# huziqi/NALO-SLAM

Hardware: AMD Instinct MI355X
Metric: keyframes/sec, KITTI-00 dense 8-KF photometric BA; pose RMSE vs ref (higher is better)
Workload: dtype f32; 1 GPU; kitti00_8kf; image=1224x368, levels=4, window_frames=8, active_points=2000, residuals=14000, tracked_frames_per_keyframe=3, multi_gpu=replicas (window too small to shard)

## Files before the change

### nalo-slam_amd/csrc/kernels_trk_lm.hip

```cpp
#include "nalo_internal.h"
#include <hip/hip_ext.h>
#include "reduce.h"
#include "trk_device.h"

namespace nalo {

constexpr int kLmThreads = 512;
constexpr int kLmStride = 56;

struct TrkLmParams {
    TrkLevel lv[NALO_MAX_LEVELS];
    double T0[12], aff0[2], ref_aff[2], minRes[5];
    float expRef, expNew;
    int coarsest, has_minres, stop_lvl, have_repeated_in;
    double* out;
    double seq;
    unsigned long long* partial;
    unsigned tag0;
};

struct LmState {
    double T[12], aff[2];
    double Tn[12], affn[2];
    double H[64], b[8], resOld[6], resNew[6];
    double lastRes[5], flow[3];
    float RKi[9], t[3], Ki[9], affa, affb, b0, cutoff, maxEnergy;
    float lambda, levelCutoffRepeat;
    int lvl, it, phase, haveRepeated, good, evals, done, break_pending, next_lvl;
    int evals_lvl[NALO_MAX_LEVELS];
};

__device__ __forceinline__ void lm_se3_exp(const double (&xi)[8], double (&T)[12]) {
    const double wx = xi[3], wy = xi[4], wz = xi[5];
    const double th2 = wx * wx + wy * wy + wz * wz;
    double qi, qr, a, bq;
    if (th2 < 0.25) {
        const double u = 0.25 * th2;
        double sc = -1.0 / 121645100408832000.0, cc = 1.0 / 6402373705728000.0;
        sc = sc * u + 1.0 / 355687428096000.0; cc = cc * u - 1.0 / 20922789888000.0;
        sc = sc * u - 1.0 / 1307674368000.0;   cc = cc * u + 1.0 / 87178291200.0;
        sc = sc * u + 1.0 / 6227020800.0;      cc = cc * u - 1.0 / 479001600.0;
        sc = sc * u - 1.0 / 39916800.0;        cc = cc * u + 1.0 / 3628800.0;
        sc = sc * u + 1.0 / 362880.0;          cc = cc * u - 1.0 / 40320.0;
        sc = sc * u - 1.0 / 5040.0;            cc = cc * u + 1.0 / 720.0;
        sc = sc * u + 1.0 / 120.0;             cc = cc * u - 1.0 / 24.0;
        sc = sc * u - 1.0 / 6.0;               cc = cc * u + 0.5;
        sc = sc * u + 1.0;                     cc = 1.0 - cc * u;
        qi = 0.5 * sc; qr = cc;
        const double v = th2;
        double pa = -1.0 / 51090942171709440000.0, pb = 1.0 / 1124000727777607680000.0;
        pa = pa * v + 1.0 / 121645100408832000.0; pb = pb * v - 1.0 / 2432902008176640000.0;
        pa = pa * v - 1.0 / 355687428096000.0;    pb = pb * v + 1.0 / 6402373705728000.0;
        pa = pa * v + 1.0 / 1307674368000.0;      pb = pb * v - 1.0 / 20922789888000.0;
        pa = pa * v - 1.0 / 6227020800.0;         pb = pb * v + 1.0 / 87178291200.0;
        pa = pa * v + 1.0 / 39916800.0;           pb = pb * v - 1.0 / 479001600.0;
        pa = pa * v - 1.0 / 362880.0;             pb = pb * v + 1.0 / 3628800.0;
        pa = pa * v + 1.0 / 5040.0;               pb = pb * v - 1.0 / 40320.0;
        pa = pa * v - 1.0 / 120.0;                pb = pb * v + 1.0 / 720.0;
        pa = pa * v + 1.0 / 6.0;                  pb = pb * v - 1.0 / 24.0;
        bq = pa; a = pb * v + 0.5;
    } else {
        const double th = sqrt(th2);
        double sh, ch;
        sincos(0.5 * th, &sh, &ch);
        qi = sh / th; qr = ch;
        a = (2.0 * sh * sh) / th2; bq = (th - 2.0 * sh * ch) / (th2 * th);
    }
    double q[4] = {qr, qi * wx, qi * wy, qi * wz};
    const double qn2 = q[0] * q[0] + q[1] * q[1] + q[2] * q[2] + q[3] * q[3];
    const double qs = 1.5 - 0.5 * qn2;
#pragma unroll
    for (int i = 0; i < 4; ++i) q[i] *= qs;
    const double w = q[0], x = q[1], y = q[2], z = q[3];
    const double R[9] = {1 - 2 * (y * y + z * z), 2 * (x * y - w * z), 2 * (x * z + w * y), 2 * (x * y + w * z), 1 - 2 * (x * x + z * z), 2 * (y * z - w * x),
                         2 * (x * z - w * y), 2 * (y * z + w * x), 1 - 2 * (x * x + y * y)};
    const double O[9] = {0, -wz, wy, wz, 0, -wx, -wy, wx, 0};
    double O2[9], V[9];
#pragma unroll
    for (int i = 0; i < 3; ++i)
#pragma unroll
        for (int j = 0; j < 3; ++j) O2[i * 3 + j] = O[i * 3] * O[j] + O[i * 3 + 1] * O[3 + j] + O[i * 3 + 2] * O[6 + j];
#pragma unroll
    for (int i = 0; i < 9; ++i) V[i] = ((i % 4 == 0) ? 1.0 : 0.0) + a * O[i] + bq * O2[i];
#pragma unroll
    for (int i = 0; i < 3; ++i) {
#pragma unroll
        for (int j = 0; j < 3; ++j) T[i * 4 + j] = R[i * 3 + j];
        T[i * 4 + 3] = V[i * 3] * xi[0] + V[i * 3 + 1] * xi[1] + V[i * 3 + 2] * xi[2];
    }
}
__device__ __forceinline__ void lm_se3_mul(const double (&A)[12], const double (&B)[12], double (&C)[12]) {
#pragma unroll
    for (int i = 0; i < 3; ++i) {
#pragma unroll
        for (int j = 0; j < 3; ++j) C[i * 4 + j] = A[i * 4] * B[j] + A[i * 4 + 1] * B[4 + j] + A[i * 4 + 2] * B[8 + j];
        C[i * 4 + 3] = A[i * 4] * B[3] + A[i * 4 + 1] * B[7] + A[i * 4 + 2] * B[11] + A[i * 4 + 3];
    }
}
__device__ __forceinline__ double lm_bcast(double v, int srclane) {
    const int lo = __builtin_amdgcn_readlane(__double2loint(v), srclane), hi = __builtin_amdgcn_readlane(__double2hiint(v), srclane);
    return __hiloint2double(hi, lo);
}
__device__ __forceinline__ void lm_wave_sync() {
    __builtin_amdgcn_fence(__ATOMIC_RELEASE, "wavefront");
    __builtin_amdgcn_wave_barrier();
    __builtin_amdgcn_fence(__ATOMIC_ACQUIRE, "wavefront");
}
__device__ __forceinline__ constexpr int lm_ut(int r, int c) { return r * 8 - r * (r - 1) / 2 + (c - r); }
__device__ __forceinline__ void lm_ldlt8_uniform(double (&U)[36], const double (&rhs)[8], double (&x)[8]) {
    double dinv[8];
#pragma unroll
    for (int k = 0; k < 8; ++k) {
        const double d = U[lm_ut(k, k)];
        const bool ok = d != 0.0 && isfinite(d);
        double rd = __builtin_amdgcn_rcp(d);
        rd = rd * (2.0 - d * rd); rd = rd * (2.0 - d * rd);
        dinv[k] = ok ? rd : 0.0;
#pragma unroll
        for (int i = k + 1; i < 8; ++i) {
            const double l = U[lm_ut(k, i)] * dinv[k];
#pragma unroll
            for (int j = i; j < 8; ++j) U[lm_ut(i, j)] -= l * U[lm_ut(k, j)];
            U[lm_ut(k, i)] = l;
        }
    }
    double y[8];
#pragma unroll
    for (int i = 0; i < 8; ++i) {
        double sacc = rhs[i];
#pragma unroll
        for (int j = 0; j < i; ++j) sacc -= U[lm_ut(j, i)] * y[j];
        y[i] = sacc;
    }
#pragma unroll
    for (int i = 7; i >= 0; --i) {
        double sacc = y[i] * dinv[i];
#pragma unroll
        for (int j = i + 1; j < 8; ++j) sacc -= U[lm_ut(i, j)] * x[j];
        x[i] = sacc;
    }
}

__device__ __forceinline__ void lm_prepare_eval(LmState& S, const TrkLmParams& P, int lvl, float levelCutoffRepeat, const double (&T)[12], double aff0, double aff1, bool write) {
    const TrkLevel& L = P.lv[lvl];
    float expF = P.expRef, expT = P.expNew;
    if (expF == 0 || expT == 0) expT = expF = 1;
    const double a = exp(aff0 - P.ref_aff[0]) * expT / expF, bq = aff1 - a * P.ref_aff[1];
    const float Ki[9] = {1.0f / L.fx, 0, -L.cx / L.fx, 0, 1.0f / L.fy, -L.cy / L.fy, 0, 0, 1};
    float Rf[9], RKi[9];
#pragma unroll
    for (int i = 0; i < 3; ++i)
#pragma unroll
        for (int j = 0; j < 3; ++j) Rf[i * 3 + j] = (float)T[i * 4 + j];
#pragma unroll
    for (int i = 0; i < 3; ++i)
#pragma unroll
        for (int j = 0; j < 3; ++j) RKi[i * 3 + j] = Rf[i * 3] * Ki[j] + Rf[i * 3 + 1] * Ki[3 + j] + Rf[i * 3 + 2] * Ki[6 + j];
    if (!write) return;
    S.affa = (float)a; S.affb = (float)bq; S.b0 = (float)P.ref_aff[1];
#pragma unroll
    for (int i = 0; i < 9; ++i) { S.RKi[i] = RKi[i]; S.Ki[i] = Ki[i]; }
#pragma unroll
    for (int i = 0; i < 3; ++i) S.t[i] = (float)T[i * 4 + 3];
    S.cutoff = kCoarseCutoffTH * levelCutoffRepeat;
    S.maxEnergy = 2 * kHuberTH * S.cutoff - kHuberTH * kHuberTH;
}
__device__ __forceinline__ double lm_scale(int r) { return r < 3 ? (double)kScaleXiRot : r < 6 ? (double)kScaleXiTrans : r == 6 ? (double)kScaleA : (double)kScaleB; }
__device__ __forceinline__ int lm_max_iterations(int lvl) { return lvl == 0 ? 10 : lvl == 1 ? 20 : 50; }
__device__ __forceinline__ unsigned long long lm_pack(float v, unsigned tag) { return ((unsigned long long)tag << 32) | (unsigned long long)__float_as_uint(v); }

__global__ __launch_bounds__(kLmThreads) void trk_lm_kernel(TrkLmParams P) {
    __shared__ float rows[(kLmThreads / 4) * kLmStride];
    __shared__ double sums[64];
    __shared__ double part[kLmThreads / 64][64];
    __shared__ LmState S;
    __shared__ int bar_ok;
    const int tid = threadIdx.x, blk = blockIdx.x, NB = gridDim.x;
    const float lambdaExtrapolationLimit = 0.001f;
    int timed_out = 0;
    if (tid == 0) bar_ok = 1;
    float c_id = 0.f, c_x = 0.f, c_y = 0.f, c_rc = 0.f;
    int cached_lvl = -1;

    if (tid == 0) {
        for (int i = 0; i < 12; ++i) S.T[i] = P.T0[i];
        S.aff[0] = P.aff0[0]; S.aff[1] = P.aff0[1];
        for (int i = 0; i < 5; ++i) S.lastRes[i] = NAN;
        S.flow[0] = S.flow[1] = S.flow[2] = 1000;
        S.lvl = P.coarsest; S.it = 0; S.phase = 0; S.next_lvl = -1; S.haveRepeated = P.have_repeated_in; S.good = 1; S.evals = 0; S.done = 0; S.break_pending = 0;
        S.levelCutoffRepeat = 1; S.lambda = 0.01f;
        for (int i = 0; i < NALO_MAX_LEVELS; ++i) S.evals_lvl[i] = 0;
        double T0[12];
#pragma unroll
        for (int i = 0; i < 12; ++i) T0[i] = P.T0[i];
        lm_prepare_eval(S, P, P.coarsest, 1.f, T0, P.aff0[0], P.aff0[1], true);
    }
    __syncthreads();

    for (int guard = 0; guard < 4096; ++guard) {
        if (S.done) break;
        const TrkLevel& L = P.lv[S.lvl];
        float acc[kTrkVals];
#pragma unroll
        for (int k = 0; k < kTrkVals; ++k) acc[k] = 0.f;
        {
            const float wlm3 = (float)(L.wl - 3), hlm3 = (float)(L.hl - 3);
            const float affa = S.affa, affb = S.affb, b0 = S.b0, cutoff = S.cutoff, maxEnergy = S.maxEnergy;
            const int lvl = S.lvl;
            float RK[9], Kq[9], tt[3];
#pragma unroll
            for (int q = 0; q < 9; ++q) { RK[q] = S.RKi[q]; Kq[q] = S.Ki[q]; }
            tt[0] = S.t[0]; tt[1] = S.t[1]; tt[2] = S.t[2];
            constexpr int G = 1;
            const int gthreads = NB * kLmThreads;
            const bool one_round = L.n <= gthreads;
            if (one_round && cached_lvl != lvl) {
                const int i = blk * kLmThreads + tid, ii = i < L.n ? i : 0;
                c_id = L.id[ii]; c_x = L.u[ii]; c_y = L.v[ii]; c_rc = L.col[ii];
                cached_lvl = lvl;
            }
            for (int base = blk * kLmThreads + tid; base < L.n; base += G * gthreads) {
                float id[G], x[G], y[G], rc[G], Ku[G], Kv[G], uu[G], vv[G], nid[G];
                bool inb[G], ok[G];
#pragma unroll
                for (int g = 0; g < G; ++g) {
                    const int i = base + g * gthreads;
                    inb[g] = i < L.n;
                    const int ii = inb[g] ? i : 0;
                    if (one_round) { id[g] = c_id; x[g] = c_x; y[g] = c_y; rc[g] = c_rc; }
                    else { id[g] = L.id[ii]; x[g] = L.u[ii]; y[g] = L.v[ii]; rc[g] = L.col[ii]; }
                }
                float4 p00[G], p10[G], p01[G], p11[G];
#pragma unroll
                for (int g = 0; g < G; ++g) {
                    trk_project(RK, tt, L, x[g], y[g], id[g], uu[g], vv[g], Ku[g], Kv[g], nid[g]);
                    ok[g] = inb[g] && (Ku[g] > 2.f && Kv[g] > 2.f && Ku[g] < wlm3 && Kv[g] < hlm3 && nid[g] > 0.f);
                    const int ix = ok[g] ? (int)Ku[g] : 2, iy = ok[g] ? (int)Kv[g] : 2;
                    const float4* bp = L.dI + ix + iy * L.wl;
                    p00[g] = bp[0]; p10[g] = bp[1]; p01[g] = bp[L.wl]; p11[g] = bp[1 + L.wl];
                }
#pragma unroll
                for (int g = 0; g < G; ++g) {
                    const int i = base + g * gthreads;
                    if (inb[g] && lvl == 0 && (i & 31) == 0) trk_flow(acc, RK, Kq, tt, L, x[g], y[g], id[g], Ku[g], Kv[g]);
                    if (!ok[g]) continue;
                    const float3 hit = trk_interp(Ku[g], Kv[g], p00[g], p10[g], p01[g], p11[g]);
                    if (!isfinite(hit.x)) continue;
                    float hw; const float residual = trk_residual(hit.x, rc[g], affa, affb, hw);
                    acc[kTrkNE] += 1.f;
                    if (fabsf(residual) > cutoff) { acc[kTrkE] += maxEnergy; acc[kTrkNSat] += 1.f; }
                    else {
                        acc[kTrkE] += hw * residual * residual * (2.f - hw);
                        acc[kTrkNWarped] += 1.f;
                        float J[9];
                        trk_jacobian(J, hit, rc[g], uu[g], vv[g], nid[g], L.fx, L.fy, affa, b0, residual);
#pragma unroll
                        for (int r = 0; r < 9; ++r) {
                            const float Jw = J[r] * hw;
#pragma unroll
                            for (int c2 = r; c2 < 9; ++c2) acc[trk_ut(r, c2)] += Jw * J[c2];
                        }
                    }
                }
            }
        }
        const int nbl = min(NB, (L.n + kLmThreads - 1) / kLmThreads);
        if (blk < nbl) {
#pragma unroll
            for (int k = 0; k < kTrkVals; ++k) acc[k] = dpp_quad_sum(acc[k]);
            if ((tid & 3) == 0) {
                float* row = rows + (tid >> 2) * kLmStride;
#pragma unroll
                for (int k = 0; k < kTrkVals; ++k) row[k] = acc[k];
            }
            __syncthreads();
            {
                const int j = tid & 63, g = tid >> 6;
                double s = 0;
                if (j < kTrkVals) for (int r = g * 16; r < g * 16 + 16; ++r) s += (double)rows[r * kLmStride + j];
                part[g][j] = s;
            }
            __syncthreads();
            if (tid < kTrkVals) {
                double s = 0; for (int g = 0; g < kLmThreads / 64; ++g) s += part[g][tid];
                if (NB == 1) sums[tid] = s;
                else __hip_atomic_store(&P.partial[((size_t)(S.evals & 1) * NB + blk) * 64 + tid], lm_pack((float)s, P.tag0 + (unsigned)S.evals), __ATOMIC_RELAXED, __HIP_MEMORY_SCOPE_AGENT);
            }
        }
        if (NB > 1) {
            const int j = tid & 63, g = tid >> 6;
            const unsigned long long* pp = P.partial + (size_t)(S.evals & 1) * NB * 64;
            const unsigned want = P.tag0 + (unsigned)S.evals;
            double s = 0;
            bool pending = j < kTrkVals;
            for (unsigned spins = 0; pending; ++spins) {
                pending = false; s = 0;
                for (int b2 = g; b2 < nbl; b2 += kLmThreads / 64) {
                    const unsigned long long wv = __hip_atomic_load(&pp[(size_t)b2 * 64 + j], __ATOMIC_RELAXED, __HIP_MEMORY_SCOPE_AGENT);
                    pending |= (unsigned)(wv >> 32) != want;
                    s += (double)__uint_as_float((unsigned)wv);
                }
                if (pending) { if (spins > (1u << 21)) { bar_ok = 0; break; } __builtin_amdgcn_s_sleep(1); }
            }
            part[g][j] = s;
            __syncthreads();
            if (!bar_ok) { timed_out = 1; break; }
            if (tid < kTrkVals) { double t2 = 0; for (int g2 = 0; g2 < kLmThreads / 64; ++g2) t2 += part[g2][tid]; sums[tid] = t2; }
        }
        __syncthreads();
        if (tid < 64) {
            const int lane = tid;
            int phase = S.phase, it = S.it, lvl = S.lvl, brk = S.break_pending, haveRep = S.haveRepeated, good = S.good, done = 0, next_lvl = S.next_lvl;
            float lambda = S.lambda, lcr = S.levelCutoffRepeat;
            const int evals = S.evals + 1;
            if (lane == 0) S.evals_lvl[S.lvl] += 1;
            const double E = sums[kTrkE], nE = sums[kTrkNE], nSat = sums[kTrkNSat], nW = sums[kTrkNWarped], sT = sums[kTrkST], sRT = sums[kTrkSRT], sN = sums[kTrkSN];
            const double st[6] = {E, nE, sT, sN, sRT, E / nE};
            const double inv = 1.0 / (double)(((long)nW + 3) & ~3L);
            const int hr = lane >> 3, hc = lane & 7, lo = hr < hc ? hr : hc, hi = hr < hc ? hc : hr;
            const double Hval = sums[lo * 9 - lo * (lo - 1) / 2 + (hi - lo)] * inv * lm_scale(hr) * lm_scale(hc);
            const int bl = lane & 7;
            const double bval = sums[bl * 9 - bl * (bl - 1) / 2 + (8 - bl)] * inv * lm_scale(bl);
            double ro[6];
#pragma unroll
            for (int i = 0; i < 6; ++i) ro[i] = S.resOld[i];
            int next_action;
            bool store_H = false, take_T = false;
            if (phase == 0) {
                store_H = true;
                if ((double)((float)nSat / (float)nE) > 0.6 && lcr < 50) { lcr *= 2; next_action = 0; }
                else { lambda = 0.01f; it = 0; brk = 0; next_action = 1; }
            } else {
                const bool accept = st[5] < ro[5];
                if (accept) { store_H = true; take_T = true; lambda *= 0.5f; }
                else { lambda *= 4; if (lambda < lambdaExtrapolationLimit) lambda = lambdaExtrapolationLimit; }
                it++;
                next_action = brk ? 2 : 1;
            }
            if (store_H) {
                S.H[lane] = Hval;
                if (lane < 8) S.b[lane] = bval;
#pragma unroll
                for (int i = 0; i < 6; ++i) ro[i] = st[i];
            }
            if (take_T) { if (lane < 12) S.T[lane] = S.Tn[lane]; else if (lane < 14) S.aff[lane - 12] = S.affn[lane - 12]; }
            lm_wave_sync();
            double T[12];
#pragma unroll
            for (int i = 0; i < 12; ++i) T[i] = S.T[i];
            const double aff0 = S.aff[0], aff1 = S.aff[1];
            if (next_action == 1) {
                if (it < lm_max_iterations(lvl)) {
                    double U[36], rhs[8], iv[8], is[8];
                    const float opl = 1 + lambda;
#pragma unroll
                    for (int r = 0; r < 8; ++r) {
#pragma unroll
                        for (int cc = r; cc < 8; ++cc) U[lm_ut(r, cc)] = S.H[r * 8 + cc];
                        U[lm_ut(r, r)] *= opl;
                        rhs[r] = -S.b[r];
                    }
                    lm_ldlt8_uniform(U, rhs, iv);
                    float extrapFac = 1;
                    if (lambda < lambdaExtrapolationLimit) extrapFac = sqrtf(sqrtf(lambdaExtrapolationLimit / lambda));
#pragma unroll
                    for (int i = 0; i < 8; ++i) { iv[i] *= extrapFac; is[i] = iv[i] * (i < 3 ? (double)kScaleXiRot : i < 6 ? (double)kScaleXiTrans : i == 6 ? (double)kScaleA : (double)kScaleB); }
                    double ssum = 0, nrm = 0;
#pragma unroll
                    for (int i = 0; i < 8; ++i) { ssum += is[i]; nrm += iv[i] * iv[i]; }
                    if (!isfinite(ssum)) {
#pragma unroll
                        for (int i = 0; i < 8; ++i) is[i] = 0;
                    }
                    double E12[12], Tn[12];
                    lm_se3_exp(is, E12);
                    lm_se3_mul(E12, T, Tn);
                    const double affn0 = aff0 + is[6], affn1 = aff1 + is[7];
                    brk = !(sqrt(nrm) > 1e-3);
                    if (lane == 0) {
#pragma unroll
                        for (int i = 0; i < 12; ++i) S.Tn[i] = Tn[i];
                        S.affn[0] = affn0; S.affn[1] = affn1;
                    }
                    lm_prepare_eval(S, P, lvl, lcr, Tn, affn0, affn1, lane == 0);
                    phase = 1;
                } else next_action = 2;
            }
            if (next_action == 0) lm_prepare_eval(S, P, lvl, lcr, T, aff0, aff1, lane == 0);
            if (next_action == 2) {
                const double lr = (double)sqrtf((float)ro[5]);
                if (lane == 0) { S.lastRes[lvl] = lr; S.flow[0] = ro[2] / (ro[3] + 0.1); S.flow[1] = 0; S.flow[2] = ro[4] / (ro[3] + 0.1); }
                if (P.has_minres && lr > 1.5 * P.minRes[lvl]) { good = 0; done = 1; }
                else {
                    int next = lvl - 1;
                    if (lcr > 1 && !haveRep) { next = lvl; haveRep = 1; }
                    if (next < P.stop_lvl) { done = 1; next_lvl = next; }
                    else { lvl = next; lcr = 1; phase = 0; lm_prepare_eval(S, P, lvl, lcr, T, aff0, aff1, lane == 0); }
                }
            }
            if (lane == 0) {
#pragma unroll
                for (int i = 0; i < 6; ++i) S.resOld[i] = ro[i];
                S.phase = phase; S.it = it; S.lvl = lvl; S.break_pending = brk; S.haveRepeated = haveRep; S.good = good; S.next_lvl = next_lvl;
                S.lambda = lambda; S.levelCutoffRepeat = lcr; S.evals = evals; S.done = done;
            }
        }
        __syncthreads();
    }
    if (blk == 0 && tid == 0) {
        double* o = P.out;
        int ok = S.good;
        for (int i = 0; i < 12; ++i) o[i] = S.T[i];
        o[12] = S.aff[0]; o[13] = S.aff[1];
        for (int i = 0; i < 5; ++i) o[14 + i] = S.lastRes[i];
        for (int i = 0; i < 3; ++i) o[19 + i] = S.flow[i];
        if (ok && (fabsf((float)S.aff[0]) > 1.2f || fabsf((float)S.aff[1]) > 200.f)) ok = 2;
        if (timed_out) ok = -1;
        for (int i = 0; i < 5; ++i) o[26 + i] = (double)S.evals_lvl[i];
        o[22] = (double)ok; o[23] = (double)S.evals; o[24] = (double)S.next_lvl; o[25] = (double)S.haveRepeated;
        __threadfence_system();
        __hip_atomic_store(&o[31], P.seq, __ATOMIC_RELEASE, __HIP_MEMORY_SCOPE_SYSTEM);
    }
}

constexpr int kLmMaxBlocks = 64;
int trk_lm_blocks(int maxn) {
    const int max_blocks = (maxn >= 8 * kLmMaxBlocks * kLmThreads ? 2 * kLmMaxBlocks : kLmMaxBlocks);
    return std::min(max_blocks, std::max(1, (maxn + kLmThreads - 1) / kLmThreads));
}

int trk_lm_launch(nalo_ctx* c, int slot_new, const double T0[12], const double aff0[2], const double ref_aff[2], const float exposures[2],
                  int coarsest, int stop_lvl, const double* minRes, double out24[32]) {
    TrkLmParams P;
    std::memset(&P, 0, sizeof(P));
    for (int l = 0; l < c->levels; ++l) P.lv[l] = trk_level(c, slot_new, l);
    std::memcpy(P.T0, T0, sizeof(P.T0)); P.aff0[0] = aff0[0]; P.aff0[1] = aff0[1]; P.ref_aff[0] = ref_aff[0]; P.ref_aff[1] = ref_aff[1];
    P.expRef = exposures[0]; P.expNew = exposures[1]; P.coarsest = coarsest; P.stop_lvl = stop_lvl; P.have_repeated_in = 0;
    P.has_minres = 0;
    if (minRes) { P.has_minres = 1; for (int i = 0; i < 5; ++i) { P.minRes[i] = minRes[i]; } }
    double* const dout = c->trk_out_host.dev;
    P.out = dout + 64;
    P.seq = (double)(++c->trk_seq);
    int maxn = 1;
    for (int l = stop_lvl; l <= coarsest; ++l) maxn = std::max(maxn, c->pc_n[l]);
    const int NB = trk_lm_blocks(maxn);
    c->trk_cfg[0] = kLmThreads; c->trk_cfg[1] = NB; c->trk_cfg[2] = 1;
    for (int l = 0; l < 5; ++l) c->trk_cfg[3 + l] = (l >= stop_lvl && l <= coarsest) ? (c->pc_n[l] + NB * kLmThreads - 1) / (NB * kLmThreads) : 0;
    if (!c->lm_partial.p || (c->lm_launches & 0xFFFFFu) == 0) {
        NALO_HIP(c, c->lm_partial.reserve((size_t)2 * 256 * 64));
        NALO_HIP(c, hipMemsetAsync(c->lm_partial.p, 0, (size_t)2 * 256 * 64 * 8, c->stream));
    }
    P.partial = c->lm_partial.p;
    P.tag0 = (unsigned)((++c->lm_launches & 0xFFFFFu) << 12);
    {
        ProfScope ps(c, "trk_lm", true);
        if (ps.a) hipExtLaunchKernelGGL(trk_lm_kernel, dim3(NB), dim3(kLmThreads), 0, c->stream, ps.a, ps.b, 0, P);
        else trk_lm_kernel<<<NB, kLmThreads, 0, c->stream>>>(P);
    }
    NALO_HIP(c, hipGetLastError());
    if (!poll_flag(c, &c->trk_out_host.p[64 + 31], P.seq)) return NALO_ERR_HIP;
    std::memcpy(out24, c->trk_out_host.p + 64, sizeof(double) * 26);
    for (int i = 0; i < 5; ++i) c->lm_evals_lvl[i] = (int)c->trk_out_host.p[64 + 26 + i];
    c->trk_cfg[8] = out24[25] != 0.0;
    if (out24[22] < 0) return NALO_LM_LOST_BLOCK;
    if (c->inject_lm_lost_block > 0 && --c->inject_lm_lost_block == 0) return NALO_LM_LOST_BLOCK;
    return NALO_OK;
}

}
```

Measured before the change: 967.0 keyframes/s.

## Split LM control step across three redundant waves with per-wave state copies

The serial Levenberg-Marquardt control step between reductions used to run on one wave, which did the 8x8 solve, the SE3 exp/multiply, the pose/K precompute, the affine exp and the bookkeeping in sequence. Now three waves each keep a private copy of the control state and repeat the cheap solve, then split the tail: wave 0 does the SE3 update and rotation-K product, wave 1 does the affine and cutoff setup, wave 2 does the break flag and bookkeeping. Tn and brk are double-buffered by eval parity so the waves need not sync with each other. The aim is a shorter serial critical path per LM iteration. The cost is redundant solve work, more shared memory, and a risk of the copies diverging.

Result: no change. 972.7 keyframes/s (median of 3 runs) (+0.6%).

```diff
diff --git a/nalo-slam_amd/csrc/kernels_trk_lm.hip b/nalo-slam_amd/csrc/kernels_trk_lm.hip
--- a/nalo-slam_amd/csrc/kernels_trk_lm.hip
+++ b/nalo-slam_amd/csrc/kernels_trk_lm.hip
@@ -19,14 +19,21 @@
     unsigned tag0;
 };
 
+constexpr int kLmCtlWaves = 3;
+struct LmCtl {
+    double T[12], aff[2];
+    double affn[2];
+    double H[64], b[8], resOld[6];
+    float lambda, levelCutoffRepeat;
+    int lvl, it, phase, haveRepeated, good, evals, next_lvl;
+};
 struct LmState {
-    double T[12], aff[2];
-    double Tn[12], affn[2];
-    double H[64], b[8], resOld[6], resNew[6];
+    double Tn[2][12];
     double lastRes[5], flow[3];
-    float RKi[9], t[3], Ki[9], affa, affb, b0, cutoff, maxEnergy;
-    float lambda, levelCutoffRepeat;
-    int lvl, it, phase, haveRepeated, good, evals, done, break_pending, next_lvl;
+    float RKi[9], t[3], Ki[9];
+    float affa, affb, b0, cutoff, maxEnergy;
+    int brk[2];
+    int lvl, evals, done;
     int evals_lvl[NALO_MAX_LEVELS];
 };
 
@@ -141,27 +148,40 @@
     }
 }
 
-__device__ __forceinline__ void lm_prepare_eval(LmState& S, const TrkLmParams& P, int lvl, float levelCutoffRepeat, const double (&T)[12], double aff0, double aff1, bool write) {
+__device__ __forceinline__ void lm_level_ki(LmState& S, const TrkLmParams& P, int lvl, float (&Ki)[9], bool write) {
     const TrkLevel& L = P.lv[lvl];
+    const float K0[9] = {1.0f / L.fx, 0, -L.cx / L.fx, 0, 1.0f / L.fy, -L.cy / L.fy, 0, 0, 1};
+#pragma unroll
+    for (int i = 0; i < 9; ++i) Ki[i] = K0[i];
+    if (!write) return;
+#pragma unroll
+    for (int i = 0; i < 9; ++i) S.Ki[i] = K0[i];
+}
+__device__ __forceinline__ void lm_load_ki(const LmState& S, float (&Ki)[9]) {
+    Ki[0] = S.Ki[0]; Ki[1] = 0; Ki[2] = S.Ki[2]; Ki[3] = 0; Ki[4] = S.Ki[4]; Ki[5] = S.Ki[5]; Ki[6] = 0; Ki[7] = 0; Ki[8] = 1;
+}
+__device__ __forceinline__ void lm_prepare_pose(LmState& S, const float (&Ki)[9], const double (&T)[12], bool write) {
+    float Rf[9], RKi[9];
+#pragma unroll
+    for (int i = 0; i < 3; ++i)
+#pragma unroll
+        for (int j = 0; j < 3; ++j) Rf[i * 3 + j] = (float)T[i * 4 + j];
+#pragma unroll
+    for (int i = 0; i < 3; ++i)
+#pragma unroll
+        for (int j = 0; j < 3; ++j) RKi[i * 3 + j] = Rf[i * 3] * Ki[j] + Rf[i * 3 + 1] * Ki[3 + j] + Rf[i * 3 + 2] * Ki[6 + j];
+    if (!write) return;
+#pragma unroll
+    for (int i = 0; i < 9; ++i) S.RKi[i] = RKi[i];
+#pragma unroll
+    for (int i = 0; i < 3; ++i) S.t[i] = (float)T[i * 4 + 3];
+}
+__device__ __forceinline__ void lm_prepare_aff(LmState& S, const TrkLmParams& P, float levelCutoffRepeat, double aff0, double aff1, bool write) {
     float expF = P.expRef, expT = P.expNew;
     if (expF == 0 || expT == 0) expT = expF = 1;
     const double a = exp(aff0 - P.ref_aff[0]) * expT / expF, bq = aff1 - a * P.ref_aff[1];
-    const float Ki[9] = {1.0f / L.fx, 0, -L.cx / L.fx, 0, 1.0f / L.fy, -L.cy / L.fy, 0, 0, 1};
-    float Rf[9], RKi[9];
-#pragma unroll
-    for (int i = 0; i < 3; ++i)
-#pragma unroll
-        for (int j = 0; j < 3; ++j) Rf[i * 3 + j] = (float)T[i * 4 + j];
-#pragma unroll
-    for (int i = 0; i < 3; ++i)
-#pragma unroll
-        for (int j = 0; j < 3; ++j) RKi[i * 3 + j] = Rf[i * 3] * Ki[j] + Rf[i * 3 + 1] * Ki[3 + j] + Rf[i * 3 + 2] * Ki[6 + j];
     if (!write) return;
     S.affa = (float)a; S.affb = (float)bq; S.b0 = (float)P.ref_aff[1];
-#pragma unroll
-    for (int i = 0; i < 9; ++i) { S.RKi[i] = RKi[i]; S.Ki[i] = Ki[i]; }
-#pragma unroll
-    for (int i = 0; i < 3; ++i) S.t[i] = (float)T[i * 4 + 3];
     S.cutoff = kCoarseCutoffTH * levelCutoffRepeat;
     S.maxEnergy = 2 * kHuberTH * S.cutoff - kHuberTH * kHuberTH;
 }
@@ -174,6 +194,7 @@
     __shared__ double sums[64];
     __shared__ double part[kLmThreads / 64][64];
     __shared__ LmState S;
+    __shared__ LmCtl ctl[kLmCtlWaves];
     __shared__ int bar_ok;
     const int tid = threadIdx.x, blk = blockIdx.x, NB = gridDim.x;
     const float lambdaExtrapolationLimit = 0.001f;
@@ -182,18 +203,28 @@
     float c_id = 0.f, c_x = 0.f, c_y = 0.f, c_rc = 0.f;
     int cached_lvl = -1;
 
-    if (tid == 0) {
-        for (int i = 0; i < 12; ++i) S.T[i] = P.T0[i];
-        S.aff[0] = P.aff0[0]; S.aff[1] = P.aff0[1];
-        for (int i = 0; i < 5; ++i) S.lastRes[i] = NAN;
-        S.flow[0] = S.flow[1] = S.flow[2] = 1000;
-        S.lvl = P.coarsest; S.it = 0; S.phase = 0; S.next_lvl = -1; S.haveRepeated = P.have_repeated_in; S.good = 1; S.evals = 0; S.done = 0; S.break_pending = 0;
-        S.levelCutoffRepeat = 1; S.lambda = 0.01f;
-        for (int i = 0; i < NALO_MAX_LEVELS; ++i) S.evals_lvl[i] = 0;
-        double T0[12];
-#pragma unroll
-        for (int i = 0; i < 12; ++i) T0[i] = P.T0[i];
-        lm_prepare_eval(S, P, P.coarsest, 1.f, T0, P.aff0[0], P.aff0[1], true);
+    if (tid < kLmCtlWaves * 64 && (tid & 63) == 0) {
+        const int wv = tid >> 6;
+        LmCtl& C = ctl[wv];
+        for (int i = 0; i < 12; ++i) C.T[i] = P.T0[i];
+        C.aff[0] = P.aff0[0]; C.aff[1] = P.aff0[1];
+        C.lvl = P.coarsest; C.it = 0; C.phase = 0; C.next_lvl = -1; C.haveRepeated = P.have_repeated_in; C.good = 1; C.evals = 0;
+        C.levelCutoffRepeat = 1; C.lambda = 0.01f;
+        if (wv == 0) {
+            double T0[12];
+#pragma unroll
+            for (int i = 0; i < 12; ++i) T0[i] = P.T0[i];
+            float Ki[9];
+            lm_level_ki(S, P, P.coarsest, Ki, true);
+            lm_prepare_pose(S, Ki, T0, true);
+        } else if (wv == 1) lm_prepare_aff(S, P, 1.f, P.aff0[0], P.aff0[1], true);
+        else {
+            for (int i = 0; i < 5; ++i) S.lastRes[i] = NAN;
+            S.flow[0] = S.flow[1] = S.flow[2] = 1000;
+            S.brk[0] = S.brk[1] = 0;
+            S.lvl = P.coarsest; S.evals = 0; S.done = 0;
+            for (int i = 0; i < NALO_MAX_LEVELS; ++i) S.evals_lvl[i] = 0;
+        }
     }
     __syncthreads();
 
@@ -308,12 +339,14 @@
             if (tid < kTrkVals) { double t2 = 0; for (int g2 = 0; g2 < kLmThreads / 64; ++g2) t2 += part[g2][tid]; sums[tid] = t2; }
         }
         __syncthreads();
-        if (tid < 64) {
-            const int lane = tid;
-            int phase = S.phase, it = S.it, lvl = S.lvl, brk = S.break_pending, haveRep = S.haveRepeated, good = S.good, done = 0, next_lvl = S.next_lvl;
-            float lambda = S.lambda, lcr = S.levelCutoffRepeat;
-            const int evals = S.evals + 1;
-            if (lane == 0) S.evals_lvl[S.lvl] += 1;
+        if (tid < kLmCtlWaves * 64) {
+            const int lane = tid & 63, wv = __builtin_amdgcn_readfirstlane(tid >> 6);
+            LmCtl& C = ctl[wv];
+            int phase = C.phase, it = C.it, lvl = C.lvl, haveRep = C.haveRepeated, good = C.good, done = 0, next_lvl = C.next_lvl;
+            float lambda = C.lambda, lcr = C.levelCutoffRepeat;
+            const int evals = C.evals + 1, par = evals & 1;
+            int brk = S.brk[par ^ 1];
+            if (wv == 2 && lane == 0) S.evals_lvl[lvl] += 1;
             const double E = sums[kTrkE], nE = sums[kTrkNE], nSat = sums[kTrkNSat], nW = sums[kTrkNWarped], sT = sums[kTrkST], sRT = sums[kTrkSRT], sN = sums[kTrkSN];
             const double st[6] = {E, nE, sT, sN, sRT, E / nE};
             const double inv = 1.0 / (double)(((long)nW + 3) & ~3L);
@@ -323,7 +356,7 @@
             const double bval = sums[bl * 9 - bl * (bl - 1) / 2 + (8 - bl)] * inv * lm_scale(bl);
             double ro[6];
 #pragma unroll
-            for (int i = 0; i < 6; ++i) ro[i] = S.resOld[i];
+            for (int i = 0; i < 6; ++i) ro[i] = C.resOld[i];
             int next_action;
             bool store_H = false, take_T = false;
             if (phase == 0) {
@@ -338,17 +371,14 @@
                 next_action = brk ? 2 : 1;
             }
             if (store_H) {
-                S.H[lane] = Hval;
-                if (lane < 8) S.b[lane] = bval;
+                C.H[lane] = Hval;
+                if (lane < 8) C.b[lane] = bval;
 #pragma unroll
                 for (int i = 0; i < 6; ++i) ro[i] = st[i];
             }
-            if (take_T) { if (lane < 12) S.T[lane] = S.Tn[lane]; else if (lane < 14) S.aff[lane - 12] = S.affn[lane - 12]; }
+            if (take_T) { if (lane < 12) C.T[lane] = S.Tn[par ^ 1][lane]; else if (lane < 14) C.aff[lane - 12] = C.affn[lane - 12]; }
             lm_wave_sync();
-            double T[12];
-#pragma unroll
-            for (int i = 0; i < 12; ++i) T[i] = S.T[i];
-            const double aff0 = S.aff[0], aff1 = S.aff[1];
+            const double aff0 = C.aff[0], aff1 = C.aff[1];
             if (next_action == 1) {
                 if (it < lm_max_iterations(lvl)) {
                     double U[36], rhs[8], iv[8], is[8];
@@ -356,9 +386,9 @@
 #pragma unroll
                     for (int r = 0; r < 8; ++r) {
 #pragma unroll
-                        for (int cc = r; cc < 8; ++cc) U[lm_ut(r, cc)] = S.H[r * 8 + cc];
+                        for (int cc = r; cc < 8; ++cc) U[lm_ut(r, cc)] = C.H[r * 8 + cc];
                         U[lm_ut(r, r)] *= opl;
-                        rhs[r] = -S.b[r];
+                        rhs[r] = -C.b[r];
                     }
                     lm_ldlt8_uniform(U, rhs, iv);
                     float extrapFac = 1;
@@ -372,52 +402,70 @@
 #pragma unroll
                         for (int i = 0; i < 8; ++i) is[i] = 0;
                     }
-                    double E12[12], Tn[12];
-                    lm_se3_exp(is, E12);
-                    lm_se3_mul(E12, T, Tn);
                     const double affn0 = aff0 + is[6], affn1 = aff1 + is[7];
-                    brk = !(sqrt(nrm) > 1e-3);
-                    if (lane == 0) {
-#pragma unroll
-                        for (int i = 0; i < 12; ++i) S.Tn[i] = Tn[i];
-                        S.affn[0] = affn0; S.affn[1] = affn1;
+                    if (lane == 0) { C.affn[0] = affn0; C.affn[1] = affn1; }
+                    if (wv == 0) {
+                        float Ki[9];
+                        lm_load_ki(S, Ki);
+                        double T[12], E12[12], Tn[12];
+#pragma unroll
+                        for (int i = 0; i < 12; ++i) T[i] = C.T[i];
+                        lm_se3_exp(is, E12);
+                        lm_se3_mul(E12, T, Tn);
+                        if (lane == 0) {
+#pragma unroll
+                            for (int i = 0; i < 12; ++i) S.Tn[par][i] = Tn[i];
+                        }
+                        lm_prepare_pose(S, Ki, Tn, lane == 0);
+                    } else if (wv == 1) lm_prepare_aff(S, P, lcr, affn0, affn1, lane == 0);
+                    else {
+                        brk = !(sqrt(nrm) > 1e-3);
+                        if (lane == 0) S.brk[par] = brk;
                     }
-                    lm_prepare_eval(S, P, lvl, lcr, Tn, affn0, affn1, lane == 0);
                     phase = 1;
                 } else next_action = 2;
             }
-            if (next_action == 0) lm_prepare_eval(S, P, lvl, lcr, T, aff0, aff1, lane == 0);
+            if (next_action == 0) {
+                if (wv == 0) { float Ki[9]; lm_load_ki(S, Ki); lm_prepare_pose(S, Ki, C.T, lane == 0); }
+                else if (wv == 1) lm_prepare_aff(S, P, lcr, aff0, aff1, lane == 0);
+            }
             if (next_action == 2) {
                 const double lr = (double)sqrtf((float)ro[5]);
-                if (lane == 0) { S.lastRes[lvl] = lr; S.flow[0] = ro[2] / (ro[3] + 0.1); S.flow[1] = 0; S.flow[2] = ro[4] / (ro[3] + 0.1); }
+                if (wv == 2 && lane == 0) { S.lastRes[lvl] = lr; S.flow[0] = ro[2] / (ro[3] + 0.1); S.flow[1] = 0; S.flow[2] = ro[4] / (ro[3] + 0.1); }
                 if (P.has_minres && lr > 1.5 * P.minRes[lvl]) { good = 0; done = 1; }
                 else {
                     int next = lvl - 1;
                     if (lcr > 1 && !haveRep) { next = lvl; haveRep = 1; }
                     if (next < P.stop_lvl) { done = 1; next_lvl = next; }
-                    else { lvl = next; lcr = 1; phase = 0; lm_prepare_eval(S, P, lvl, lcr, T, aff0, aff1, lane == 0); }
+                    else {
+                        lvl = next; lcr = 1; phase = 0;
+                        if (wv == 0) { float Ki[9]; lm_level_ki(S, P, lvl, Ki, lane == 0); lm_prepare_pose(S, Ki, C.T, lane == 0); }
+                        else if (wv == 1) lm_prepare_aff(S, P, lcr, aff0, aff1, lane == 0);
+                    }
                 }
             }
             if (lane == 0) {
 #pragma unroll
-                for (int i = 0; i < 6; ++i) S.resOld[i] = ro[i];
-                S.phase = phase; S.it = it; S.lvl = lvl; S.break_pending = brk; S.haveRepeated = haveRep; S.good = good; S.next_lvl = next_lvl;
-                S.lambda = lambda; S.levelCutoffRepeat = lcr; S.evals = evals; S.done = done;
+                for (int i = 0; i < 6; ++i) C.resOld[i] = ro[i];
+                C.phase = phase; C.it = it; C.lvl = lvl; C.haveRepeated = haveRep; C.good = good; C.next_lvl = next_lvl;
+                C.lambda = lambda; C.levelCutoffRepeat = lcr; C.evals = evals;
+                if (wv == 2) { S.lvl = lvl; S.evals = evals; S.done = done; }
             }
         }
         __syncthreads();
     }
     if (blk == 0 && tid == 0) {
         double* o = P.out;
-        int ok = S.good;
-        for (int i = 0; i < 12; ++i) o[i] = S.T[i];
-        o[12] = S.aff[0]; o[13] = S.aff[1];
+        const LmCtl& C = ctl[0];
+        int ok = C.good;
+        for (int i = 0; i < 12; ++i) o[i] = C.T[i];
+        o[12] = C.aff[0]; o[13] = C.aff[1];
         for (int i = 0; i < 5; ++i) o[14 + i] = S.lastRes[i];
         for (int i = 0; i < 3; ++i) o[19 + i] = S.flow[i];
-        if (ok && (fabsf((float)S.aff[0]) > 1.2f || fabsf((float)S.aff[1]) > 200.f)) ok = 2;
+        if (ok && (fabsf((float)C.aff[0]) > 1.2f || fabsf((float)C.aff[1]) > 200.f)) ok = 2;
         if (timed_out) ok = -1;
         for (int i = 0; i < 5; ++i) o[26 + i] = (double)S.evals_lvl[i];
-        o[22] = (double)ok; o[23] = (double)S.evals; o[24] = (double)S.next_lvl; o[25] = (double)S.haveRepeated;
+        o[22] = (double)ok; o[23] = (double)C.evals; o[24] = (double)C.next_lvl; o[25] = (double)C.haveRepeated;
         __threadfence_system();
         __hip_atomic_store(&o[31], P.seq, __ATOMIC_RELEASE, __HIP_MEMORY_SCOPE_SYSTEM);
     }
```
